# JuliaParallel/DistributedArrays.jl

Hardware: NVIDIA H100
Metric: GB/s for map! and sum on Float32 DArray (higher is better)
Workload: dtype f32

## Files before the change

### distributedarrays.jl_b200/_broadcast.py

```python
from __future__ import annotations

import ctypes as C
import struct
from typing import Callable, List, Optional, Sequence, Tuple

import numpy as np

from builtins import any as builtins_any

from . import _lib
from ._darray import B200Array, DArray, dab_dtype, darray, makelocal
from .layout import shape_of
from .runtime import close_remote_reads, open_remote_reads, runtime

_RANK = {"bool": 0, "i32": 1, "i64": 2, "i128": 3, "f32": 4, "f64": 5}


class _TagTypes(dict):

    def __missing__(self, tag):
        raise _lib.UnsupportedError(_lib.ERR_UNSUPPORTED, f"values of type {tag} have no array element type on the GPU backend "
                                    "(Int128 is served as the value type of mapreduce(f, op, d) only)")


_NPT = _TagTypes({"bool": np.dtype(np.bool_), "i32": np.dtype(np.int32), "i64": np.dtype(np.int64), "f32": np.dtype(np.float32),
                  "f64": np.dtype(np.float64), "c64": np.dtype(np.complex64), "c128": np.dtype(np.complex128)})
_TAG = {v: k for k, v in _NPT.items()}
SLICE_TRACING = [0]
_CT = {"bool": "bool", "i32": "int", "i64": "long long", "i128": "i128", "f32": "float", "f64": "double", "c64": "jl_c64", "c128": "jl_c128"}
_COMP = {"c64": "f32", "c128": "f64"}
_CPLX_OF = {"f32": "c64", "f64": "c128"}


def is_ctag(t: str) -> bool:
    return t in _COMP


def tag_of(dtype) -> str:
    dt = np.dtype(dtype)
    if dt not in _TAG:
        raise _lib.UnsupportedError(_lib.ERR_UNSUPPORTED, f"element type {dt} not served by the GPU backend")
    return _TAG[dt]


def promote(a: str, b: str) -> str:
    if a == b:
        return a
    if is_ctag(a) or is_ctag(b):
        if "i128" in (a, b):
            raise _lib.UnsupportedError(_lib.ERR_UNSUPPORTED, "Int128 values mixed with complex values are not served")
        return _CPLX_OF[promote(_COMP.get(a, a), _COMP.get(b, b))]
    if "f" in a[0] + b[0]:
        fl = [t for t in (a, b) if t[0] == "f"]
        return "f64" if "f64" in fl else "f32"
    return a if _RANK[a] >= _RANK[b] else b


class Expr:

    __slots__ = ("op", "args", "jt", "val", "weak")
    __array_ufunc__ = None

    def __init__(self, op, args=(), jt="f64", val=None, weak=False):
        self.op, self.args, self.jt, self.val, self.weak = op, tuple(args), jt, val, weak
# ... 354 lines not shown
        return unop("inv", inner(x))
    f.__name__ = name
    return f


def _mk_of_inv(name, outer):
    def f(x):
        if not isinstance(x, Expr):
            raise TypeError(f"dab.{name} is for use inside broadcast/map kernels")
        return outer(unop("inv", x))
    f.__name__ = name
    return f


sec, csc, cot = _mk_inv_of("sec", cos), _mk_inv_of("csc", sin), _mk_inv_of("cot", tan)
sech, csch, coth = _mk_inv_of("sech", cosh), _mk_inv_of("csch", sinh), _mk_inv_of("coth", tanh)
asec, acsc, acot = _mk_of_inv("asec", acos), _mk_of_inv("acsc", asin), _mk_of_inv("acot", atan)
asech, acsch, acoth = _mk_of_inv("asech", acosh), _mk_of_inv("acsch", asinh), _mk_of_inv("acoth", atanh)


def _float_of(x: Expr) -> Expr:
    return x if x.jt[0] == "f" else convert(x, "f64")


def deg2rad(x):
    x = _float_of(Expr.wrap(x))
    t = _NPT[x.jt].type
    return binop("mul", x, Expr("const", (), x.jt, float(t(np.pi) / t(180))))


def rad2deg(x):
    x = _float_of(Expr.wrap(x))
    t = _NPT[x.jt].type
    return binop("mul", x, Expr("const", (), x.jt, float(t(180) / t(np.pi))))


def jl_max(a, b):
    return binop("max", Expr.wrap(a), Expr.wrap(b))


def jl_min(a, b):
    return binop("min", Expr.wrap(a), Expr.wrap(b))


def mod(a, b):
    return binop("mod", Expr.wrap(a), Expr.wrap(b))


def rem(a, b):
    return binop("rem", Expr.wrap(a), Expr.wrap(b))


def trace(f: Callable, arg_tags: Sequence[str]) -> Expr:
    syms = [Expr("arg", (), t, k) for k, t in enumerate(arg_tags)]
    return Expr.wrap(f(*syms))


_FN2 = {"add": "jl_add", "sub": "jl_sub", "mul": "jl_mul", "div": "jl_div", "rem": "jl_rem", "mod": "jl_mod", "idiv": "jl_idiv",
        "max": "jl_max", "min": "jl_min", "pow": "jl_pow", "and": "jl_and", "or": "jl_or", "xor": "jl_xor", "lt": "jl_lt", "le": "jl_le",
        "gt": "jl_gt", "ge": "jl_ge", "eq": "jl_eq", "ne": "jl_ne", "x_shl": "jl_x_shl", "x_shr": "jl_x_shr"}
_FN2.update({"m_copysign": "jl_m_copysign", "m_powi": "jl_m_powi"})
_FN2.update({"m_" + c: "jl_m_" + c for c in ("lt", "le", "gt", "ge", "eq", "ne")})


def _lit(jt: str, v) -> str:
    if jt == "f32":
        return "__int_as_float((int)0x%08x)" % struct.unpack("<I", struct.pack("<f", float(v)))[0]
    if jt == "f64":
        return "__longlong_as_double((long long)0x%016xULL)" % struct.unpack("<Q", struct.pack("<d", float(v)))[0]
    if is_ctag(jt):
        z = complex(v)
        return "%s(%s, %s)" % (_CT[jt], _lit(_COMP[jt], z.real), _lit(_COMP[jt], z.imag))
    if jt == "i32":
        return "((int)%d)" % int(v)
    if jt == "i64":
        return "((long long)%dLL)" % int(v)
    if jt == "i128":
        v = int(v) % (1 << 128)
        return "((i128)(((u128)0x%016xULL << 64) | (u128)0x%016xULL))" % (v >> 64, v & ((1 << 64) - 1))
    return "true" if v else "false"


def codegen(e: Expr) -> str:
    if e.op == "arg":
        return f"a{e.val}"
    if e.op == "const":
        return _lit(e.jt, e.val)
    if e.op == "convert":
        if is_ctag(e.jt):
            return f"{_CT[e.jt]}({codegen(e.args[0])})"
        return f"(({_CT[e.jt]})({codegen(e.args[0])}))"
    if e.op == "complex":
        return f"{_CT[e.jt]}({codegen(e.args[0])}, {codegen(e.args[1])})"
    if e.op == "ifelse":
        return f"(({codegen(e.args[0])}) ? ({codegen(e.args[1])}) : ({codegen(e.args[2])}))"
    if e.op in _FN2:
        return f"{_FN2[e.op]}({codegen(e.args[0])}, {codegen(e.args[1])})"
    return f"jl_{e.op}({codegen(e.args[0])})"


_UN = {"abs": _lib.MAP_ABS, "abs2": _lib.MAP_ABS2, "neg": _lib.MAP_NEG, "sqrt": _lib.MAP_SQRT, "inv": _lib.MAP_INV,
       "floor": _lib.MAP_FLOOR, "ceil": _lib.MAP_CEIL, "sign": _lib.MAP_SIGN}
_BIN = {"add": _lib.ADD, "sub": _lib.SUB, "mul": _lib.MUL, "div": _lib.DIV, "rem": _lib.REM, "max": _lib.BMAX, "min": _lib.BMIN,
        "mod": _lib.MOD, "idiv": _lib.IDIV, "and": _lib.AND, "or": _lib.OR, "xor": _lib.XOR}


def _is_arg(e: Expr, k=None):
    return e.op == "arg" and (k is None or e.val == k)


def match_affine(e: Expr):
    def lin(t):
        if _is_arg(t, 0):
            return 1
        if t.op == "mul":
            l, r = t.args
            if l.op == "const" and _is_arg(r, 0):
                return l.val
            if r.op == "const" and _is_arg(l, 0):
                return r.val
        return None

    if e.op == "add":
        l, r = e.args
        if r.op == "const" and lin(l) is not None:
            return lin(l), r.val
        if l.op == "const" and lin(r) is not None:
            return lin(r), l.val
    return None


def _pad4(v, fill=1):
    v = list(v)
    if len(v) > 4:
        raise _lib.UnsupportedError(_lib.ERR_UNSUPPORTED, "broadcast whose dimensions do not collapse to 4 groups (see collapse_dims) is not served")
    return v + [fill] * (4 - len(v))


def collapse_dims(out_shape, arg_shapes):
    nd = len(out_shape)
    shapes = [tuple(int(v) for v in sh) + (1,) * (nd - len(sh)) for sh in arg_shapes]
    groups: List[Tuple[int, List[int]]] = []
    for d in range(nd):
        o = int(out_shape[d])
        ext = [sh[d] for sh in shapes]
        for e, sh in zip(ext, arg_shapes):
            if e != o and e != 1:
                raise _lib.DimensionMismatch(_lib.ERR_DIM_MISMATCH, f"arrays could not be broadcast: {tuple(sh)} vs {tuple(out_shape)}")
        if o == 1:
            continue
        if groups:
            po, pext = groups[-1]
            if all((pe == po and e == o) or (pe == 1 and e == 1) for pe, e in zip(pext, ext)):
                groups[-1] = (po * o, [pe * e for pe, e in zip(pext, ext)])
                continue
        groups.append((o, ext))
    if not groups:
        groups = [(1, [1] * len(shapes))]
    return tuple(g[0] for g in groups), [tuple(g[1][k] for g in groups) for k in range(len(shapes))]


def _dense_strides(shape):
    s, out = 1, []
    for d in shape:
        out.append(s)
        s *= int(d)
    return out


class LocalArg:

    def __init__(self, arr: Optional[B200Array] = None, scalar=None, tag: str = "f64", temp: bool = False):
        self.arr, self.scalar, self.tag, self.temp = arr, scalar, tag, temp


def run_local(rt, expr: Expr, out: B200Array, largs: List[LocalArg]):
    n = out.size
    if n == 0:
        return
    out_tag = tag_of(out.dtype)
    full = [a for a in largs if a.arr is not None]
    same = all(a.arr.shape == out.shape or a.arr.size == n and _squeeze(a.arr.shape) == _squeeze(out.shape) for a in full)
    ctx = rt.ctx
    code = dab_dtype(out.dtype)
    rt.last_kernel = "fixed"
    cplx = uses_complex(expr) or builtins_any(is_ctag(a.tag) for a in largs)
    if same and not cplx and expr.jt == out_tag and out_tag != "bool":
        x0 = largs[0] if largs and largs[0].arr is not None and largs[0].tag == out_tag else None
        if x0 is not None and all(_only_arg0(expr)):
            ab = match_affine(expr)
            if ab is not None:
                a = np.asarray(ab[0], dtype=out.dtype)
                b = np.asarray(ab[1], dtype=out.dtype)
                _lib.call("dab_affine", ctx, code, C.c_void_p(out.ptr), C.c_void_p(x0.arr.ptr), C.c_void_p(a.ctypes.data),
                          C.c_void_p(b.ctypes.data), n)
                rt.last_kernel = "dab_affine"
                return
            if expr.op in _UN and _is_arg(expr.args[0], 0):
                _lib.call("dab_unary", ctx, code, _UN[expr.op], C.c_void_p(out.ptr), C.c_void_p(x0.arr.ptr), n)
                return
            if _is_arg(expr, 0):
                _lib.call("dab_unary", ctx, code, _lib.MAP_ID, C.c_void_p(out.ptr), C.c_void_p(x0.arr.ptr), n)
                return
        if expr.op in _BIN and len(expr.args) == 2 and not (expr.op == "div" and out_tag[0] != "f"):
            l, r = expr.args
            la = largs[l.val] if l.op == "arg" else None
            ra = largs[r.val] if r.op == "arg" else None

            def arr_ok(e, a):
                return e.op == "arg" and a is not None and a.arr is not None and a.tag == out_tag

            def sc_val(e, a):
                if e.op == "const" and e.jt == out_tag:
                    return e.val
                if e.op == "arg" and a is not None and a.arr is None and a.tag == out_tag:
                    return a.scalar
                return None

            if arr_ok(l, la) and arr_ok(r, ra):
                _lib.call("dab_binary", ctx, code, _BIN[expr.op], C.c_void_p(out.ptr), C.c_void_p(la.arr.ptr), C.c_void_p(ra.arr.ptr), n)
                return
            if arr_ok(l, la) and sc_val(r, ra) is not None:
                s = np.asarray(sc_val(r, ra), dtype=out.dtype)
                _lib.call("dab_binary_scalar", ctx, code, _BIN[expr.op], C.c_void_p(out.ptr), C.c_void_p(la.arr.ptr), C.c_void_p(s.ctypes.data), 0, n)
                return
            if arr_ok(r, ra) and sc_val(l, la) is not None:
                s = np.asarray(sc_val(l, la), dtype=out.dtype)
                _lib.call("dab_binary_scalar", ctx, code, _BIN[expr.op], C.c_void_p(out.ptr), C.c_void_p(ra.arr.ptr), C.c_void_p(s.ctypes.data), 1, n)
                return
    if expr.op == "const" and expr.jt == out_tag:
        v = np.asarray(expr.val, dtype=out.dtype)
        _lib.call("dab_fill", ctx, code, C.c_void_p(out.ptr), n, C.c_void_p(v.ctypes.data))
        return
    rt.last_kernel = "dab_broadcast_expr"
    if uses_tag(expr, "i128"):
        raise _lib.UnsupportedError(_lib.ERR_UNSUPPORTED, "Int128 values are served inside mapreduce(f, op, d) only, not in a broadcast")
    if expr.jt[0] == "f" and out_tag[0] not in "fc":
        raise _lib.UnsupportedError(_lib.ERR_UNSUPPORTED, f"broadcast of {expr.jt} values into a {out_tag} destination (InexactError semantics) is not served")
    if is_ctag(expr.jt) and not is_ctag(out_tag):
        raise _lib.UnsupportedError(_lib.ERR_UNSUPPORTED, f"broadcast of {expr.jt} values into a {out_tag} destination (InexactError semantics) is not served")
    expr, largs = split_c128_scalars(expr, largs)
    src = codegen(convert(expr, out_tag)).encode()
    oshape_nd, ashapes = tuple(out.shape), {k: tuple(a.arr.shape) for k, a in enumerate(largs) if a.arr is not None}
    if len(oshape_nd) > 4 or any(len(sh) > 4 for sh in ashapes.values()):
        keys = sorted(ashapes)
        oshape_nd, coll = collapse_dims(oshape_nd, [ashapes[k] for k in keys])
        ashapes = dict(zip(keys, coll))
    oshape = _pad4(oshape_nd)
    nargs = len(largs)
    if nargs > 8:
# ... 62 lines not shown
        ext = 1
        for s in shapes:
            v = s[k] if k < len(s) else 1
            if v != 1:
                if ext != 1 and ext != v:
                    raise _lib.DimensionMismatch(_lib.ERR_DIM_MISMATCH, f"arrays could not be broadcast to a common size: {shapes}")
                ext = v
        out.append(ext)
    return tuple(out)


def _arg_tag(a) -> str:
    if isinstance(a, (DArray,)):
        return tag_of(a.dtype)
    if isinstance(a, np.ndarray) and a.ndim > 0:
        return tag_of(a.dtype)
    return Expr.wrap(a.item() if isinstance(a, np.ndarray) else a).jt


def _bcview(arg_dims: Sequence[int], I) -> Tuple:
    out = []
    for k, s in enumerate(arg_dims):
        if s == 1:
            out.append((1, 1))
        elif k < len(I):
            lo, hi = I[k]
            if not (1 <= lo and hi <= s):
                raise _lib.DimensionMismatch(_lib.ERR_DIM_MISMATCH, "broadcast view could not be constructed")
            out.append((lo, hi))
        else:
            out.append((1, s))
    return tuple(out)


def _localise(rt, a, I, pid) -> LocalArg:
    if isinstance(a, DArray):
        view = _bcview(a.dims, I)
        arr = makelocal(a, view, pid)
        return LocalArg(arr, None, tag_of(a.dtype), temp=arr is not a.chunks.get(pid))
    if isinstance(a, np.ndarray) and a.ndim > 0:
        view = _bcview(a.shape, I)
        sl = a[tuple(slice(lo - 1, hi) for lo, hi in view)]
        return LocalArg(B200Array.from_numpy(rt, sl), None, tag_of(a.dtype), temp=True)
    e = Expr.wrap(a.item() if isinstance(a, np.ndarray) else a)
    return LocalArg(None, e.val, e.jt)


def _remote_args(dest_layout, args) -> List[DArray]:
    return [a for a in args if isinstance(a, DArray) and not (a.layout.pids == dest_layout.pids and a.layout.indices == dest_layout.indices)]


def _broadcast_chunks(dest: DArray, expr: Expr, args) -> DArray:
    rt = dest.rt
    fenced = open_remote_reads(rt, _remote_args(dest.layout, args), "host")
    for pid, out in dest.chunks.items():
        I = dest.layout.localindices(pid)
        largs = [_localise(rt, a, I, pid) for a in args]
        run_local(rt, expr, out, largs)
        for la in largs:
            if la.temp and la.arr is not None:
                la.arr.free()
    close_remote_reads(rt, fenced, "host")
    return dest


def _materialise_views(args):
    from ._darray import SubDArray
    out, temps = [], []
    for a in args:
        if isinstance(a, SubDArray):
            a = a.to_darray()
            temps.append(a)
        out.append(a)
    return out, temps


def broadcast_into(dest: DArray, f: Callable, *args) -> DArray:
    args, _views = _materialise_views(args)
    try:
        return _broadcast_into(dest, f, *args)
    finally:
        for v in _views:
            v.close()


def _broadcast_into(dest: DArray, f: Callable, *args) -> DArray:
    shapes = [a.dims if isinstance(a, DArray) else (a.shape if isinstance(a, np.ndarray) else ()) for a in args]
    for shp in shapes:
        for k, s in enumerate(shp):
            want = dest.dims[k] if k < len(dest.dims) else 1
            if s != 1 and s != want:
                raise _lib.DimensionMismatch(_lib.ERR_DIM_MISMATCH, f"destination axes {dest.dims} are not compatible with source axes {tuple(shp)}")
    expr = trace(f, [_arg_tag(a) for a in args])
    return _broadcast_chunks(dest, expr, args)


def broadcast(f: Callable, *args, rt=None) -> DArray:
    args, _views = _materialise_views(args)
    try:
        return _broadcast(f, *args, rt=rt)
    finally:
        for v in _views:
            v.close()


def _broadcast(f: Callable, *args, rt=None) -> DArray:
    rt = rt or next((a.rt for a in args if isinstance(a, DArray)), None) or runtime()
    shapes = [a.dims if isinstance(a, DArray) else (a.shape if isinstance(a, np.ndarray) else ()) for a in args]
    dims = _bc_shape(shapes)
    expr = trace(f, [_arg_tag(a) for a in args])
    out_dt = _NPT[expr.jt]
    dest = darray(lambda I: B200Array.empty(rt, shape_of(I), out_dt), dims, dtype=out_dt, rt=rt)
    return _broadcast_chunks(dest, expr, args)


def copy(d: DArray) -> DArray:
    from ._darray import similar
    return _broadcast_into(similar(d), lambda x: x, d)


# ... 68 lines not shown
```

### distributedarrays.jl_b200/_darray.py

```python
from __future__ import annotations

import ctypes as C
import itertools
import weakref
from typing import Callable, Dict, List, Optional, Sequence, Tuple

import numpy as np

from . import _lib
from .layout import Layout, Range, default_procs, layout_from_chunk_shapes, make_layout, rlen, shape_of, slab_plan
from .runtime import Runtime, close_remote_reads, open_remote_reads, runtime

_DT = {np.dtype(np.float32): _lib.F32, np.dtype(np.float64): _lib.F64, np.dtype(np.int32): _lib.I32,
       np.dtype(np.int64): _lib.I64, np.dtype(np.bool_): _lib.U8,
       np.dtype(np.complex64): _lib.C64, np.dtype(np.complex128): _lib.C128}
_NP = {_lib.F32: np.dtype(np.float32), _lib.F64: np.dtype(np.float64), _lib.I32: np.dtype(np.int32),
       _lib.I64: np.dtype(np.int64), _lib.U8: np.dtype(np.bool_), _lib.C64: np.dtype(np.complex64), _lib.C128: np.dtype(np.complex128)}


def dab_dtype(dt) -> int:
    dt = np.dtype(dt)
    if dt not in _DT:
        raise _lib.UnsupportedError(_lib.ERR_UNSUPPORTED, f"element type {dt} is not served by the GPU backend (no host fallback)")
    return _DT[dt]


def np_dtype(code: int) -> np.dtype:
    return _NP[code]


def is_complex(dt) -> bool:
    return np.dtype(dt).kind == "c"


def component_dtype(dt) -> np.dtype:
    dt = np.dtype(dt)
    return {np.dtype(np.complex64): np.dtype(np.float32), np.dtype(np.complex128): np.dtype(np.float64)}.get(dt, dt)


_allowscalar = [True]


def allowscalar(flag: bool = True):
    _allowscalar[0] = bool(flag)


class B200Array:

    __slots__ = ("rt", "ptr", "shape", "dtype", "_own", "_keep", "_temp")

    def __init__(self, rt: Runtime, ptr: int, shape: Sequence[int], dtype, own: bool = True, keep=None, temp: bool = False):
        self.rt, self.ptr, self.shape, self.dtype = rt, int(ptr), tuple(int(s) for s in shape), np.dtype(dtype)
        self._own, self._keep, self._temp = own, keep, temp

    @classmethod
    def empty(cls, rt: Runtime, shape: Sequence[int], dtype, temp: bool = False) -> "B200Array":
        dtype = np.dtype(dtype)
        n = int(np.prod(shape)) if len(shape) else 1
        ptr = rt.alloc_temp(n * dtype.itemsize) if temp else rt.alloc(n * dtype.itemsize)
        return cls(rt, ptr, shape, dtype, temp=temp)

    @classmethod
    def from_numpy(cls, rt: Runtime, a: np.ndarray) -> "B200Array":
        a = np.asarray(a)
        dab_dtype(a.dtype)
        out = cls.empty(rt, a.shape, a.dtype)
        out.copy_from_host(a)
        return out

    @property
    def size(self) -> int:
        return int(np.prod(self.shape)) if len(self.shape) else 1

    @property
    def nbytes(self) -> int:
        return self.size * self.dtype.itemsize

    @property
    def ndim(self) -> int:
        return len(self.shape)

    def copy_from_host(self, a: np.ndarray, sync: bool = True):
        a = np.asarray(a, dtype=self.dtype)
        if tuple(a.shape) != self.shape:
            raise _lib.DimensionMismatch(_lib.ERR_DIM_MISMATCH, f"host array {a.shape} vs chunk {self.shape}")
        if self.size == 0:
            return
        if not a.flags.f_contiguous:
            if a.ndim == 2 and a.strides[0] == a.itemsize and a.strides[1] > 0:
                _lib.call("dab_h2d_2d", self.rt.ctx, C.c_void_p(self.ptr), a.shape[0] * a.itemsize, C.c_void_p(a.ctypes.data),
                          a.strides[1], a.shape[0] * a.itemsize, a.shape[1])
                if sync:
                    self.rt.sync()
                return
            a = np.asfortranarray(a)
        _lib.call("dab_h2d", self.rt.ctx, C.c_void_p(self.ptr), C.c_void_p(a.ctypes.data), self.nbytes)
        if sync:
            self.rt.sync()

    def to_numpy(self) -> np.ndarray:
        out = np.empty(self.shape, dtype=self.dtype, order="F")
        if self.size:
            _lib.call("dab_d2h", self.rt.ctx, C.c_void_p(out.ctypes.data), C.c_void_p(self.ptr), self.nbytes)
            self.rt.sync()
        return out

    def free(self):
        if self._own and self.ptr:
            if self._temp:
                self.rt.free_temp(self.ptr)
            else:
                self.rt.free(self.ptr)
        self.ptr = 0

    def __repr__(self):
        return f"B200Array({self.dtype}, {self.shape}, ptr=0x{self.ptr:x}, dev={self.rt.device})"


def pinned_empty(rt: Runtime, shape, dtype) -> np.ndarray:
    dtype = np.dtype(dtype)
    n = int(np.prod(shape)) if len(shape) else 1
    p = C.c_void_p()
    _lib.call("dab_host_alloc", rt.ctx, max(1, n * dtype.itemsize), C.byref(p))
    buf = (C.c_char * max(1, n * dtype.itemsize)).from_address(p.value)
    arr = np.frombuffer(buf, dtype=dtype, count=n).reshape(shape, order="F")
# ... 627 lines not shown
```

### distributedarrays.jl_b200/_mapreduce.py

```python
from __future__ import annotations

import builtins
import ctypes as C
import operator
from itertools import accumulate
from typing import Callable, Dict, Optional, Sequence, Tuple

import numpy as np

from . import _lib
from ._broadcast import Expr, broadcast, is_ctag, tag_of, trace, _NPT
from ._darray import B200Array, DArray, component_dtype, dab_dtype, is_complex, np_dtype
from .layout import Layout, ravel, reduction_passes, shape_of, unravel
from .runtime import close_remote_reads, deliver, exchange_stacks, open_remote_reads

_OPS = {"+": _lib.SUM, "add": _lib.SUM, "sum": _lib.SUM, "*": _lib.PROD, "mul": _lib.PROD, "prod": _lib.PROD, "max": _lib.MAX,
        "min": _lib.MIN}
_OPF = {operator.add: _lib.SUM, operator.mul: _lib.PROD, builtins.max: _lib.MAX, builtins.min: _lib.MIN, np.add: _lib.SUM,
        np.multiply: _lib.PROD, np.maximum: _lib.MAX, np.minimum: _lib.MIN}


def _op_code(op) -> int:
    if isinstance(op, str) and op in _OPS:
        return _OPS[op]
    if op in _OPF:
        return _OPF[op]
    raise _lib.UnsupportedError(_lib.ERR_UNSUPPORTED, f"reduction operator {op!r} is not served by a kernel (no host fallback)")


_CMPMAP = {"eq": _lib.MAP_EQ, "ne": _lib.MAP_NE, "lt": _lib.MAP_LT, "le": _lib.MAP_LE, "gt": _lib.MAP_GT, "ge": _lib.MAP_GE}
_FLIP = {"lt": "gt", "le": "ge", "gt": "lt", "ge": "le", "eq": "eq", "ne": "ne"}


def classify_map(f: Optional[Callable], dtype) -> Tuple[Optional[int], Optional[np.ndarray], Optional[Expr]]:
    if f is None:
        return _lib.MAP_ID, None, None
    tag = tag_of(dtype)
    e = trace(f, [tag])
    if e.op == "arg":
        return _lib.MAP_ID, None, e
    if is_ctag(tag):
        if len(e.args) == 1 and e.args[0].op == "arg":
            code = {"abs": _lib.MAP_ABS, "abs2": _lib.MAP_ABS2, "neg": _lib.MAP_NEG, "isnan": _lib.MAP_ISNAN}.get(e.op)
            if code is not None:
                return code, None, e
        return None, None, e
    if e.jt == tag and len(e.args) == 1 and e.args[0].op == "arg":
        code = {"abs": _lib.MAP_ABS, "abs2": _lib.MAP_ABS2, "neg": _lib.MAP_NEG}.get(e.op)
        if code is not None:
            return code, None, e
    if e.op == "mul" and e.jt == tag and builtins.all(a.op == "arg" for a in e.args):
        return _lib.MAP_ABS2, None, e
    if e.op in _CMPMAP:
        l, r = e.args

        def unpromote(side, const):
            if side.op == "convert" and side.args[0].op == "arg" and side.args[0].jt == tag and const.op == "const":
                c = const.val
                if tag == "f32" and const.jt == "f64" and float(np.float32(c)) == c:
                    return side.args[0], Expr("const", (), tag, c)
                if tag in ("i32", "i64") and const.jt in ("i64",) and side.jt == "i64":
                    return side.args[0], Expr("const", (), tag, c) if -2**31 <= c < 2**31 or tag == "i64" else (side, const)
            return side, const

        l, r = unpromote(l, r)
        r, l = unpromote(r, l)
        if l.op == "arg" and r.op == "const" and l.jt == tag:
            return _CMPMAP[e.op], np.asarray(r.val, dtype=np.dtype(dtype)), e
        if r.op == "arg" and l.op == "const" and r.jt == tag:
            return _CMPMAP[_FLIP[e.op]], np.asarray(l.val, dtype=np.dtype(dtype)), e
    if e.op == "isnan" and e.args[0].op == "arg":
        return _lib.MAP_ISNAN, None, e
    return None, None, e


def _result_dtype(dtype, op: int, mapc: int) -> np.dtype:
    out = C.c_int32()
    _lib.check(_lib.lib().dab_reduce_result_dtype(dab_dtype(dtype), op, mapc, C.byref(out)))
    return np.dtype(np.int64) if out.value == _lib.I64 else np_dtype(out.value)




def _gather_slots(d: DArray, launch: Callable[[int, B200Array, int], None]) -> np.ndarray:
    rt = d.rt
    wpr = rt.workers_per_rank
    slots = B200Array.empty(rt, (16 * wpr,), np.uint8, temp=True)
    try:
        for pid, ch in d.chunks.items():
            launch(pid, ch, slots.ptr + 16 * ((pid - 1) % wpr))
        if rt.world > 1:
            allslots = B200Array.empty(rt, (16 * wpr * rt.world,), np.uint8, temp=True)
            _lib.call("dab_allgather", rt.ctx, C.c_void_p(slots.ptr), C.c_void_p(allslots.ptr), 16 * wpr)
            host = allslots.to_numpy()
            allslots.free()
        else:
            host = slots.to_numpy()
    finally:
        rt.sync()
        slots.free()
    return host.view(np.uint8)


def _fold(host: np.ndarray, pids: Sequence[int], rdt: np.dtype, op: int):
    vals = np.empty(len(pids), dtype=rdt)
    for i, pid in enumerate(pids):
        vals[i] = host[16 * (pid - 1):16 * (pid - 1) + rdt.itemsize].view(rdt)[0]
    out = np.zeros(1, dtype=rdt)
    rcode = _lib.I64 if rdt == np.dtype(np.int64) else dab_dtype(rdt)
    _lib.check(_lib.lib().dab_combine_ordered(rcode, op, C.c_void_p(vals.ctypes.data), len(pids), C.c_void_p(out.ctypes.data)))
    return out[0], vals


def _int128(b: bytes) -> int:
    return int.from_bytes(b, "little", signed=True)


def wrap128(v: int) -> int:
    v &= (1 << 128) - 1
    return v - (1 << 128) if v >> 127 else v


def fold128(vals: Sequence[int], op: int) -> int:
    acc = vals[0]
    for v in vals[1:]:
        acc = wrap128(acc + v) if op == _lib.SUM else wrap128(acc * v) if op == _lib.PROD else (max(acc, v) if op == _lib.MAX else min(acc, v))
    return acc


# ... 520 lines not shown
```

### distributedarrays.jl_b200/csrc/dab_comm.cu

```cuda
#include <dlfcn.h>
#include <nccl.h>

#include "dab_common.cuh"
#include "dab_scalar_ops.cuh"

namespace {

struct NcclApi {
    void* handle = nullptr;
    ncclResult_t (*GetUniqueId)(ncclUniqueId*) = nullptr;
    ncclResult_t (*CommInitRank)(ncclComm_t*, int, ncclUniqueId, int) = nullptr;
    ncclResult_t (*CommDestroy)(ncclComm_t) = nullptr;
    ncclResult_t (*AllGather)(const void*, void*, size_t, ncclDataType_t, ncclComm_t, cudaStream_t) = nullptr;
    ncclResult_t (*AllReduce)(const void*, void*, size_t, ncclDataType_t, ncclRedOp_t, ncclComm_t, cudaStream_t) = nullptr;
    ncclResult_t (*Send)(const void*, size_t, ncclDataType_t, int, ncclComm_t, cudaStream_t) = nullptr;
    ncclResult_t (*Recv)(void*, size_t, ncclDataType_t, int, ncclComm_t, cudaStream_t) = nullptr;
    ncclResult_t (*GroupStart)() = nullptr;
    ncclResult_t (*GroupEnd)() = nullptr;
    const char* (*GetErrorString)(ncclResult_t) = nullptr;
    const char* (*GetLastError)(ncclComm_t) = nullptr;
    bool ok = false;
    char why[256] = "";
};

// ... 152 lines not shown
    }
    ncclRedOp_t ro;
    switch (op) {
        case DAB_SUM: ro = ncclSum; break;
        case DAB_PROD: ro = ncclProd; break;
        case DAB_MAX: ro = ncclMax; break;
        case DAB_MIN: ro = ncclMin; break;
        default: return dab_fail(ctx, DAB_ERR_ARG, "dab_allreduce: bad op %d", op);
    }
    DAB_NCCL(ctx, api.AllReduce(send_dev, recv_dev, count, dt, ro, (ncclComm_t)ctx->comm, ctx->stream));
    ctx->launches++;
    return DAB_OK;
}

int32_t dab_group_start(dab_ctx* ctx) {
    DAB_ENTER(ctx);
    NEED_COMM(ctx);
    DAB_NCCL(ctx, api.GroupStart());
    return DAB_OK;
}
int32_t dab_group_end(dab_ctx* ctx) {
    DAB_ENTER(ctx);
    NEED_COMM(ctx);
    DAB_NCCL(ctx, api.GroupEnd());
    ctx->launches++;
    return DAB_OK;
}
int32_t dab_send(dab_ctx* ctx, const void* send_dev, size_t nbytes, int32_t peer) {
    DAB_ENTER(ctx);
    NEED_COMM(ctx);
    DAB_NCCL(ctx, api.Send(send_dev, nbytes, ncclInt8, peer, (ncclComm_t)ctx->comm, ctx->stream));
    return DAB_OK;
}
int32_t dab_recv(dab_ctx* ctx, void* recv_dev, size_t nbytes, int32_t peer) {
    DAB_ENTER(ctx);
    NEED_COMM(ctx);
    DAB_NCCL(ctx, api.Recv(recv_dev, nbytes, ncclInt8, peer, (ncclComm_t)ctx->comm, ctx->stream));
    return DAB_OK;
}

int32_t dab_mapreduce_all(dab_ctx* ctx, int32_t dtype, int32_t op, int32_t map, const void* map_param, const void* x, size_t n,
                          void* out_host) {
    DAB_ENTER_NOFLUSH(ctx);
    int32_t rdt;
    if (!out_host || op == DAB_EXTREMA || dab_reduce_result_dtype(dtype, op, map, &rdt) != DAB_OK) {
        DAB_FLUSH(ctx);
        DAB_REQUIRE(ctx, out_host, DAB_ERR_ARG, "dab_mapreduce_all: null out");
        if (op == DAB_EXTREMA) return dab_fail(ctx, DAB_ERR_UNSUPPORTED, "dab_mapreduce_all: extrema combines through dab_reduce + dab_allgather");
        return dab_fail(ctx, DAB_ERR_ARG, "bad dtype/op");
    }
    const bool cplx = rdt == DAB_C64 || rdt == DAB_C128;
    if ((ctx->mbox_ranks > 1 || !ctx->comm || ctx->nranks == 1) && n > 0 && !cplx) {
        ctx->fuse_op = op;
        int32_t st = dab_reduce(ctx, dtype, op, map, map_param, x, n, ctx->result_slot);
        ctx->fuse_op = -1;
        if (st != DAB_OK) return st;
        DAB_CUDA(ctx, cudaStreamSynchronize(ctx->stream));
        const volatile unsigned long long* h = (const volatile unsigned long long*)ctx->host_slot;
        if (h[1] != 0) return dab_fail(ctx, DAB_ERR_NCCL, "fused combine timed out waiting for a peer's chunk result (did every rank call?)");
        unsigned long long bits = h[0];
        memset(out_host, 0, 8);
        memcpy(out_host, &bits, dab_dtype_size(rdt));
        return DAB_OK;
    }
    if (cplx && ctx->mbox_ranks > 1 && !ctx->comm) {
        DAB_FLUSH(ctx);
        return dab_fail(ctx, DAB_ERR_UNSUPPORTED, "dab_mapreduce_all: a complex result across %d ranks needs the NCCL communicator "
                        "(the mailbox combine carries 8-byte results)", ctx->mbox_ranks);
    }
    int32_t st = dab_reduce(ctx, dtype, op, map, map_param, x, n, ctx->result_slot);
    if (st != DAB_OK) return st;
    const int P = ctx->comm ? ctx->nranks : 1;
    const void* src = ctx->result_slot;
    if (P > 1) {
        NEED_COMM(ctx);
        DAB_NCCL(ctx, api.AllGather(ctx->result_slot, ctx->gather_slots, 16, ncclInt8, (ncclComm_t)ctx->comm, ctx->stream));
        ctx->launches++;
        src = ctx->gather_slots;
    }
    DAB_CUDA(ctx, cudaMemcpyAsync(ctx->host_slot, src, (size_t)P * 16, cudaMemcpyDeviceToHost, ctx->stream));
    DAB_CUDA(ctx, cudaStreamSynchronize(ctx->stream));
    unsigned char tmp[DAB_MAX_RANKS * 16];
    size_t es = dab_dtype_size(rdt);
    for (int i = 0; i < P; ++i) memcpy(tmp + (size_t)i * es, (const char*)ctx->host_slot + (size_t)i * 16, es);
    unsigned char res[16] = {0};
    st = dab_combine_ordered(rdt, op, tmp, (size_t)P, res);
    if (st != DAB_OK) return dab_fail(ctx, st, "%s", dab_last_error(nullptr));
    memset(out_host, 0, es > 8 ? es : 8);
    memcpy(out_host, res, es);
    return DAB_OK;
}

int32_t dab_mailbox_create(dab_ctx* ctx, void* handle64) {
    DAB_ENTER(ctx);
    DAB_REQUIRE(ctx, handle64, DAB_ERR_ARG, "dab_mailbox_create: null handle");
    if (!ctx->mailbox) {
        DAB_CUDA(ctx, cudaMalloc(&ctx->mailbox, DAB_MBOX_BYTES));
        DAB_CUDA(ctx, cudaMemset(ctx->mailbox, 0, DAB_MBOX_BYTES));
    }
    cudaIpcMemHandle_t h;
    DAB_CUDA(ctx, cudaIpcGetMemHandle(&h, ctx->mailbox));
    memcpy(handle64, &h, 64);
    return DAB_OK;
}

int32_t dab_mailbox_attach(dab_ctx* ctx, const void* handles, int32_t rank, int32_t nranks) {
    DAB_ENTER(ctx);
    DAB_REQUIRE(ctx, handles && nranks >= 1 && nranks <= DAB_MAX_RANKS && rank >= 0 && rank < nranks, DAB_ERR_ARG, "dab_mailbox_attach: bad arguments");
    DAB_REQUIRE(ctx, ctx->mailbox, DAB_ERR_ARG, "dab_mailbox_attach: call dab_mailbox_create first");
    DAB_REQUIRE(ctx, ctx->mbox_ranks == 0, DAB_ERR_ARG, "mailboxes already attached");
    for (int j = 0; j < nranks; ++j) {
        if (j == rank) {
            ctx->peer_mbox_host[j] = ctx->mailbox;
            continue;
        }
        cudaIpcMemHandle_t h;
        memcpy(&h, (const char*)handles + (size_t)j * 64, 64);
        DAB_CUDA(ctx, cudaIpcOpenMemHandle(&ctx->peer_mbox_host[j], h, cudaIpcMemLazyEnablePeerAccess));
    }
    DAB_CUDA(ctx, cudaMalloc((void**)&ctx->peer_mbox_dev, sizeof(void*) * DAB_MAX_RANKS));
    DAB_CUDA(ctx, cudaMemcpy(ctx->peer_mbox_dev, ctx->peer_mbox_host, sizeof(void*) * nranks, cudaMemcpyHostToDevice));
    ctx->rank = rank;
    ctx->mbox_ranks = nranks;
// ... 94 lines not shown
```

### distributedarrays.jl_b200/csrc/dab_common.cuh

```cuda
#pragma once
#include <cuda_runtime.h>

#include <cstdint>
#include <cstdio>
#include <cstring>

#include "../../include/dab200.h"

#define DAB_MAX_REDUCE_BLOCKS 262144
#define DAB_SLOT_BYTES 64
#define DAB_MAX_RANKS 64

struct dab_pending_affine {
    int active;
    int32_t dtype;
    void* y;
    const void* x;
    size_t n;
    unsigned char a[8], b[8];
};

struct dab_ctx {
    int device;
    int sm_count;
// ... 31 lines not shown
    long long opt_combine_timeout_ms;
    long long opt_gemm_kc;
    int opt_gemm_rawhi;
    int opt_gemm_simt;
    int opt_gemv_phase;
    int opt_gemv_t_cols;
    int opt_gemv_t_waves;
    int opt_spmv_group;
    int opt_ew_tma;
    dab_pending_affine pending;
    int defer_off;
    char err[512];
};

extern thread_local char dab_tls_err[512];

int32_t dab_fail(dab_ctx* ctx, int32_t status, const char* fmt, ...);
int32_t dab_fail_cuda(dab_ctx* ctx, cudaError_t e, const char* what, const char* file, int line);

#define DAB_CUDA(ctx, call)                                                             \
    do {                                                                                \
        cudaError_t e__ = (call);                                                       \
        if (e__ != cudaSuccess) return dab_fail_cuda((ctx), e__, #call, __FILE__, __LINE__); \
    } while (0)

#define DAB_REQUIRE(ctx, cond, status, ...)                          \
    do {                                                             \
        if (!(cond)) return dab_fail((ctx), (status), __VA_ARGS__);  \
    } while (0)

int32_t dab_flush_pending(dab_ctx* ctx);

#define DAB_FLUSH(ctx)                                    \
    do {                                                  \
        if ((ctx)->pending.active) {                      \
            int32_t st__ = dab_flush_pending(ctx);        \
            if (st__ != DAB_OK) return st__;              \
        }                                                 \
    } while (0)

#define DAB_ENTER(ctx)                                                      \
    do {                                                                    \
        if ((ctx) == nullptr) return dab_fail(nullptr, DAB_ERR_ARG, "null ctx"); \
        DAB_CUDA((ctx), cudaSetDevice((ctx)->device));                      \
        DAB_FLUSH(ctx);                                                     \
    } while (0)

#define DAB_ENTER_NOFLUSH(ctx)                                              \
    do {                                                                    \
        if ((ctx) == nullptr) return dab_fail(nullptr, DAB_ERR_ARG, "null ctx"); \
        DAB_CUDA((ctx), cudaSetDevice((ctx)->device));                      \
    } while (0)

#define DAB_LAUNCHED(ctx)                          \
    do {                                           \
        (ctx)->launches++;                         \
        DAB_CUDA((ctx), cudaGetLastError());       \
    } while (0)

int32_t dab_scratch_grow(dab_ctx* ctx, void** buf, size_t* have, size_t bytes, bool zero);

static inline size_t dab_dtype_size(int32_t dt) {
    switch (dt) {
        case DAB_F32: return 4;
        case DAB_F64: return 8;
        case DAB_I32: return 4;
        case DAB_I64: return 8;
        case DAB_U8: return 1;
        case DAB_C64: return 8;
        case DAB_C128: return 16;
        default: return 0;
    }
}

#define DAB_MBOX_SLOT 32
#define DAB_MBOX_BARRIER_OFFSET (2 * DAB_MAX_RANKS * DAB_MBOX_SLOT)
#define DAB_MBOX_BYTES (DAB_MBOX_BARRIER_OFFSET + DAB_MAX_RANKS * 8)
struct FusedComm {
    void* const* peers;
    void* host_out;
    unsigned long long seq;
    unsigned long long timeout_ns;
    int rank, nranks, op;
};

__device__ __forceinline__ unsigned long long dab_globaltimer_ns() {
    unsigned long long t;
    asm volatile("mov.u64 %0, %globaltimer;" : "=l"(t));
    return t;
}
__device__ __forceinline__ int4 ld_stream(const int4* p) { return __ldcs(p); }
__device__ __forceinline__ void st_stream(int4* p, int4 v) { __stcs(p, v); }

template <typename T>
struct alignas(16) Pack {
    static constexpr int N = 16 / sizeof(T);
    T v[N];
};

template <typename T>
struct alignas(2 * sizeof(T)) Cplx {
    T re, im;
};

template <typename T>
__device__ __forceinline__ Pack<T> as_pack(int4 r) {
// ... 32 lines not shown
```

### distributedarrays.jl_b200/csrc/dab_reduce.cu

```cuda
#include <type_traits>

#include <cmath>

#include "dab_reduce_traits.cuh"

namespace {

struct NoStore {
    template <typename T>
    __device__ __forceinline__ void vec(Pack<T>&, size_t) const {}
    template <typename T>
    __device__ __forceinline__ T scalar(T v, size_t) const { return v; }
};
template <typename T>
struct AffineStore {
    AffineF<T> f;
    T* y;
    int4* yv;
    __device__ __forceinline__ void vec(Pack<T>& p, size_t i) const {
#pragma unroll
        for (int k = 0; k < Pack<T>::N; ++k) p.v[k] = f(p.v[k]);
        st_stream(yv + i, as_int4(p));
    }
    __device__ __forceinline__ T scalar(T v, size_t i) const {
// ... 342 lines not shown
                memcpy(buf, one, 16);
            } else {
                long long one = 1;
                memcpy(buf, &one, 8);
            }
            if (flt) {
                double one = 1.0;
                memcpy(buf + 8, &one, 8);
            }
            break;
        default: return dab_fail(ctx, DAB_ERR_EMPTY, "reducing over an empty collection is not allowed");
    }
    memcpy((char*)ctx->host_slot + DAB_MAX_RANKS * 16, buf, 16);
    DAB_CUDA(ctx, cudaMemcpyAsync(out_dev, (char*)ctx->host_slot + DAB_MAX_RANKS * 16, 16, cudaMemcpyHostToDevice, ctx->stream));
    DAB_CUDA(ctx, cudaStreamSynchronize(ctx->stream));
    return DAB_OK;
}

}

extern "C" {

int32_t dab_reduce_result_dtype(int32_t dtype, int32_t op, int32_t map, int32_t* out_dtype) {
    if (!out_dtype) return DAB_ERR_ARG;
    if (dtype == DAB_C64 || dtype == DAB_C128) {
        const int32_t comp = dtype == DAB_C64 ? DAB_F32 : DAB_F64;
        const bool id = map == DAB_MAP_ID || map == DAB_MAP_NEG, mag = map == DAB_MAP_ABS || map == DAB_MAP_ABS2;
        const bool pred = map == DAB_MAP_NONZERO || map == DAB_MAP_ISNAN;
        if (id && (op == DAB_SUM || op == DAB_PROD)) *out_dtype = dtype;
        else if (mag && (op == DAB_SUM || op == DAB_MAX || op == DAB_MIN)) *out_dtype = comp;
        else if (pred && (op == DAB_SUM || op == DAB_COUNT || op == DAB_ALL || op == DAB_ANY)) *out_dtype = DAB_I64;
        else return dab_fail(nullptr, DAB_ERR_UNSUPPORTED, "op %d with map %d is not served for complex dtype %d", op, map, dtype);
        return DAB_OK;
    }
    const bool pred = map >= DAB_MAP_EQ;
    switch (op) {
        case DAB_SUM:
        case DAB_PROD:
            *out_dtype = (!pred && (dtype == DAB_F32 || dtype == DAB_F64)) ? dtype : DAB_I64;
            return DAB_OK;
        case DAB_MAX:
        case DAB_MIN:
        case DAB_EXTREMA: *out_dtype = dtype; return DAB_OK;
        case DAB_ALL:
        case DAB_ANY:
        case DAB_COUNT: *out_dtype = DAB_I64; return DAB_OK;
        default: return DAB_ERR_ARG;
    }
}

int32_t dab_reduce(dab_ctx* ctx, int32_t dtype, int32_t op, int32_t map, const void* map_param, const void* x, size_t n,
                   void* out_dev) {
    DAB_ENTER_NOFLUSH(ctx);
    if (out_dev && consumes_pending(ctx, dtype, op, map, x, n)) {
        const dab_pending_affine p = ctx->pending;
        ctx->pending.active = 0;
        switch (dtype) {
            case DAB_F32: return reduce_pending_affine<float>(ctx, op, p, out_dev);
            case DAB_F64: return reduce_pending_affine<double>(ctx, op, p, out_dev);
            case DAB_I32: return reduce_pending_affine<int32_t>(ctx, op, p, out_dev);
            default: return reduce_pending_affine<long long>(ctx, op, p, out_dev);
        }
    }
    DAB_FLUSH(ctx);
    DAB_REQUIRE(ctx, out_dev && (x || n == 0), DAB_ERR_ARG, "dab_reduce: null pointer");
    DAB_REQUIRE(ctx, op >= DAB_SUM && op <= DAB_EXTREMA, DAB_ERR_ARG, "dab_reduce: bad op %d", op);
    if (dtype == DAB_C64 || dtype == DAB_C128) {
        int32_t rdt;
        if (dab_reduce_result_dtype(dtype, op, map, &rdt) != DAB_OK)
            return dab_fail(ctx, DAB_ERR_UNSUPPORTED, "dab_reduce: op %d with map %d is not served for complex dtype %d (no host fallback)", op,
                            map, dtype);
        if (n == 0) return empty_result(ctx, map == DAB_MAP_ABS || map == DAB_MAP_ABS2 ? rdt : dtype, op, out_dev);
        if (dtype == DAB_C64) return reduce_c<float>(ctx, dtype, op, map, (const Cplx<float>*)x, n, out_dev);
        return reduce_c<double>(ctx, dtype, op, map, (const Cplx<double>*)x, n, out_dev);
    }
    if (n == 0) return empty_result(ctx, dtype, op, out_dev);
    switch (dtype) {
        case DAB_F32: return reduce_t<float>(ctx, op, map, map_param, (const float*)x, n, out_dev);
        case DAB_F64: return reduce_t<double>(ctx, op, map, map_param, (const double*)x, n, out_dev);
        case DAB_I32: return reduce_t<int32_t>(ctx, op, map, map_param, (const int32_t*)x, n, out_dev);
        case DAB_I64: return reduce_t<long long>(ctx, op, map, map_param, (const long long*)x, n, out_dev);
        case DAB_U8: return reduce_u8(ctx, op, map, (const uint8_t*)x, n, out_dev);
        default: return dab_fail(ctx, DAB_ERR_ARG, "dab_reduce: bad dtype %d", dtype);
    }
}

int32_t dab_reduce_host(dab_ctx* ctx, int32_t dtype, int32_t op, int32_t map, const void* map_param, const void* x, size_t n,
                        void* out_host) {
    DAB_ENTER_NOFLUSH(ctx);
    if (!out_host) {
        DAB_FLUSH(ctx);
        return dab_fail(ctx, DAB_ERR_ARG, "dab_reduce_host: null out");
    }
    int32_t st = dab_reduce(ctx, dtype, op, map, map_param, x, n, ctx->result_slot);
    if (st != DAB_OK) return st;
    DAB_CUDA(ctx, cudaMemcpyAsync(ctx->host_slot, ctx->result_slot, 16, cudaMemcpyDeviceToHost, ctx->stream));
    DAB_CUDA(ctx, cudaStreamSynchronize(ctx->stream));
    memcpy(out_host, ctx->host_slot, 16);
    return DAB_OK;
}

int32_t dab_combine_ordered(int32_t rdt, int32_t op, const void* partials, size_t p, void* out) {
    if (!partials || !out) return dab_fail(nullptr, DAB_ERR_ARG, "dab_combine_ordered: null pointer");
    if (p == 0) return dab_fail(nullptr, DAB_ERR_EMPTY, "reducing over an empty collection is not allowed");
#define FOLD(T, EXPR)                          \
    {                                          \
        const T* v = (const T*)partials;       \
        T a = v[0];                            \
        for (size_t i = 1; i < p; ++i) {       \
            T b = v[i];                        \
            a = (EXPR);                        \
        }                                      \
        *(T*)out = a;                          \
        return DAB_OK;                         \
    }
    auto fmax_jl = [](auto a, auto b) {
        using T = decltype(a);
        if (a != a || b != b) return (T)NAN;
        if (a == b) return std::signbit(a) ? b : a;
        return a > b ? a : b;
    };
    auto fmin_jl = [](auto a, auto b) {
        using T = decltype(a);
        if (a != a || b != b) return (T)NAN;
        if (a == b) return std::signbit(a) ? a : b;
        return a < b ? a : b;
    };
    switch (rdt) {
        case DAB_F32:
            switch (op) {
                case DAB_SUM: {
                    const float* v = (const float*)partials;
                    volatile float a = v[0];
                    for (size_t i = 1; i < p; ++i) a = a + v[i];
                    *(float*)out = a;
                    return DAB_OK;
                }
                case DAB_PROD: {
                    const float* v = (const float*)partials;
                    volatile float a = v[0];
                    for (size_t i = 1; i < p; ++i) a = a * v[i];
                    *(float*)out = a;
                    return DAB_OK;
                }
                case DAB_MAX: FOLD(float, fmax_jl(a, b))
                case DAB_MIN: FOLD(float, fmin_jl(a, b))
                default: break;
// ... 85 lines not shown
```

Baseline: 4008.

## Trim host-side overhead in broadcast and reduce dispatch paths

Caches traced expressions for closures whose captured values are plain numbers, and tries the affine kernel before the costlier complex-usage scan. It also skips the remote-read fence on a single rank, short-circuits view materialisation, memoises result dtype lookups and uses math.prod for size. A dab_reduce_entered entry avoids re-entering the context guard on nested calls. The aim is to cut Python and C entry overhead per map!/sum call, at the cost of added cache-key logic that could mis-key closures.

Measured after the change: 4122 (median of 6 runs). 2.8% higher.

```diff
diff --git a/distributedarrays.jl_b200/_broadcast.py b/distributedarrays.jl_b200/_broadcast.py
--- a/distributedarrays.jl_b200/_broadcast.py
+++ b/distributedarrays.jl_b200/_broadcast.py
@@ -2,6 +2,8 @@
 
 import ctypes as C
 import struct
+from collections import OrderedDict
+from types import CodeType, FunctionType
 from typing import Callable, List, Optional, Sequence, Tuple
 
 import numpy as np
@@ -9,7 +11,7 @@
 from builtins import any as builtins_any
 
 from . import _lib
-from ._darray import B200Array, DArray, dab_dtype, darray, makelocal
+from ._darray import B200Array, DArray, SubDArray, dab_dtype, darray, makelocal
 from .layout import shape_of
 from .runtime import close_remote_reads, open_remote_reads, runtime
 
@@ -470,8 +472,49 @@
 
 
 def trace(f: Callable, arg_tags: Sequence[str]) -> Expr:
+    key = _closed_key(f, arg_tags)
+    if key is not None:
+        e = _TRACES.get(key)
+        if e is not None:
+            _TRACES.move_to_end(key)
+            return e
     syms = [Expr("arg", (), t, k) for k, t in enumerate(arg_tags)]
-    return Expr.wrap(f(*syms))
+    e = Expr.wrap(f(*syms))
+    if key is not None:
+        _TRACES[key] = e
+        if len(_TRACES) > _TRACES_MAX:
+            _TRACES.popitem(last=False)
+    return e
+
+
+_TRACES: "OrderedDict[tuple, Expr]" = OrderedDict()
+_TRACES_MAX = 64
+_CELL_TYPES = frozenset({bool, int, float, complex} | {t for t in np.sctypeDict.values() if issubclass(t, (np.number, np.bool_))})
+
+
+def _closed_key(f, arg_tags) -> Optional[tuple]:
+    if type(f) is not FunctionType or f.__defaults__ or f.__kwdefaults__ or SLICE_TRACING[0]:
+        return None
+    code = f.__code__
+    if code.co_names or builtins_any(isinstance(c, CodeType) for c in code.co_consts):
+        return None
+    cells = []
+    for cell in f.__closure__ or ():
+        try:
+            v = cell.cell_contents
+        except ValueError:
+            return None
+        t = type(v)
+        if t not in _CELL_TYPES:
+            return None
+        if t is float:
+            v = struct.pack("<d", v)
+        elif t is complex:
+            v = struct.pack("<dd", v.real, v.imag)
+        elif t is not int and t is not bool:
+            v = v.tobytes()
+        cells.append((t, v))
+    return (code, tuple(arg_tags), tuple(cells))
 
 
 _FN2 = {"add": "jl_add", "sub": "jl_sub", "mul": "jl_mul", "div": "jl_div", "rem": "jl_rem", "mod": "jl_mod", "idiv": "jl_idiv",
@@ -530,17 +573,21 @@
 def match_affine(e: Expr):
     def lin(t):
         if _is_arg(t, 0):
-            return 1
-        if t.op == "mul":
+            return None if is_ctag(t.jt) else 1
+        if t.op == "mul" and not is_ctag(t.jt):
             l, r = t.args
+            if is_ctag(l.jt) or is_ctag(r.jt):
+                return None
             if l.op == "const" and _is_arg(r, 0):
                 return l.val
             if r.op == "const" and _is_arg(l, 0):
                 return r.val
         return None
 
-    if e.op == "add":
+    if e.op == "add" and not is_ctag(e.jt):
         l, r = e.args
+        if is_ctag(l.jt) or is_ctag(r.jt):
+            return None
         if r.op == "const" and lin(l) is not None:
             return lin(l), r.val
         if l.op == "const" and lin(r) is not None:
@@ -602,18 +649,21 @@
     ctx = rt.ctx
     code = dab_dtype(out.dtype)
     rt.last_kernel = "fixed"
-    cplx = uses_complex(expr) or builtins_any(is_ctag(a.tag) for a in largs)
-    if same and not cplx and expr.jt == out_tag and out_tag != "bool":
-        x0 = largs[0] if largs and largs[0].arr is not None and largs[0].tag == out_tag else None
+    cplx_args = builtins_any(is_ctag(a.tag) for a in largs)
+    fixed = same and expr.jt == out_tag and out_tag != "bool"
+    x0 = largs[0] if largs and largs[0].arr is not None and largs[0].tag == out_tag else None
+    if fixed and x0 is not None and not cplx_args:
+        ab = match_affine(expr)
+        if ab is not None:
+            a = np.asarray(ab[0], dtype=out.dtype)
+            b = np.asarray(ab[1], dtype=out.dtype)
+            _lib.call("dab_affine", ctx, code, C.c_void_p(out.ptr), C.c_void_p(x0.arr.ptr), C.c_void_p(a.ctypes.data),
+                      C.c_void_p(b.ctypes.data), n)
+            rt.last_kernel = "dab_affine"
+            return
+    cplx = cplx_args or uses_complex(expr)
+    if fixed and not cplx:
         if x0 is not None and all(_only_arg0(expr)):
-            ab = match_affine(expr)
-            if ab is not None:
-                a = np.asarray(ab[0], dtype=out.dtype)
-                b = np.asarray(ab[1], dtype=out.dtype)
-                _lib.call("dab_affine", ctx, code, C.c_void_p(out.ptr), C.c_void_p(x0.arr.ptr), C.c_void_p(a.ctypes.data),
-                          C.c_void_p(b.ctypes.data), n)
-                rt.last_kernel = "dab_affine"
-                return
             if expr.op in _UN and _is_arg(expr.args[0], 0):
                 _lib.call("dab_unary", ctx, code, _UN[expr.op], C.c_void_p(out.ptr), C.c_void_p(x0.arr.ptr), n)
                 return
@@ -782,7 +832,7 @@
 
 def _broadcast_chunks(dest: DArray, expr: Expr, args) -> DArray:
     rt = dest.rt
-    fenced = open_remote_reads(rt, _remote_args(dest.layout, args), "host")
+    fenced = rt.world > 1 and open_remote_reads(rt, _remote_args(dest.layout, args), "host")
     for pid, out in dest.chunks.items():
         I = dest.layout.localindices(pid)
         largs = [_localise(rt, a, I, pid) for a in args]
@@ -795,7 +845,8 @@
 
 
 def _materialise_views(args):
-    from ._darray import SubDArray
+    if not builtins_any(isinstance(a, SubDArray) for a in args):
+        return args, ()
     out, temps = [], []
     for a in args:
         if isinstance(a, SubDArray):
diff --git a/distributedarrays.jl_b200/_darray.py b/distributedarrays.jl_b200/_darray.py
--- a/distributedarrays.jl_b200/_darray.py
+++ b/distributedarrays.jl_b200/_darray.py
@@ -2,6 +2,7 @@
 
 import ctypes as C
 import itertools
+import math
 import weakref
 from typing import Callable, Dict, List, Optional, Sequence, Tuple
 
@@ -70,7 +71,7 @@
 
     @property
     def size(self) -> int:
-        return int(np.prod(self.shape)) if len(self.shape) else 1
+        return math.prod(self.shape)
 
     @property
     def nbytes(self) -> int:
diff --git a/distributedarrays.jl_b200/_mapreduce.py b/distributedarrays.jl_b200/_mapreduce.py
--- a/distributedarrays.jl_b200/_mapreduce.py
+++ b/distributedarrays.jl_b200/_mapreduce.py
@@ -2,6 +2,7 @@
 
 import builtins
 import ctypes as C
+import functools
 import operator
 from itertools import accumulate
 from typing import Callable, Dict, Optional, Sequence, Tuple
@@ -74,7 +75,8 @@
     return None, None, e
 
 
-def _result_dtype(dtype, op: int, mapc: int) -> np.dtype:
+@functools.lru_cache(maxsize=None)
+def _result_dtype(dtype: np.dtype, op: int, mapc: int) -> np.dtype:
     out = C.c_int32()
     _lib.check(_lib.lib().dab_reduce_result_dtype(dab_dtype(dtype), op, mapc, C.byref(out)))
     return np.dtype(np.int64) if out.value == _lib.I64 else np_dtype(out.value)
diff --git a/distributedarrays.jl_b200/csrc/dab_comm.cu b/distributedarrays.jl_b200/csrc/dab_comm.cu
--- a/distributedarrays.jl_b200/csrc/dab_comm.cu
+++ b/distributedarrays.jl_b200/csrc/dab_comm.cu
@@ -228,7 +228,7 @@
     const bool cplx = rdt == DAB_C64 || rdt == DAB_C128;
     if ((ctx->mbox_ranks > 1 || !ctx->comm || ctx->nranks == 1) && n > 0 && !cplx) {
         ctx->fuse_op = op;
-        int32_t st = dab_reduce(ctx, dtype, op, map, map_param, x, n, ctx->result_slot);
+        int32_t st = dab_reduce_entered(ctx, dtype, op, map, map_param, x, n, ctx->result_slot);
         ctx->fuse_op = -1;
         if (st != DAB_OK) return st;
         DAB_CUDA(ctx, cudaStreamSynchronize(ctx->stream));
@@ -244,7 +244,7 @@
         return dab_fail(ctx, DAB_ERR_UNSUPPORTED, "dab_mapreduce_all: a complex result across %d ranks needs the NCCL communicator "
                         "(the mailbox combine carries 8-byte results)", ctx->mbox_ranks);
     }
-    int32_t st = dab_reduce(ctx, dtype, op, map, map_param, x, n, ctx->result_slot);
+    int32_t st = dab_reduce_entered(ctx, dtype, op, map, map_param, x, n, ctx->result_slot);
     if (st != DAB_OK) return st;
     const int P = ctx->comm ? ctx->nranks : 1;
     const void* src = ctx->result_slot;
diff --git a/distributedarrays.jl_b200/csrc/dab_common.cuh b/distributedarrays.jl_b200/csrc/dab_common.cuh
--- a/distributedarrays.jl_b200/csrc/dab_common.cuh
+++ b/distributedarrays.jl_b200/csrc/dab_common.cuh
@@ -107,6 +107,9 @@
         DAB_CUDA((ctx), cudaSetDevice((ctx)->device));                      \
     } while (0)
 
+int32_t dab_reduce_entered(dab_ctx* ctx, int32_t dtype, int32_t op, int32_t map, const void* map_param, const void* x, size_t n,
+                           void* out_dev);
+
 #define DAB_LAUNCHED(ctx)                          \
     do {                                           \
         (ctx)->launches++;                         \
diff --git a/distributedarrays.jl_b200/csrc/dab_reduce.cu b/distributedarrays.jl_b200/csrc/dab_reduce.cu
--- a/distributedarrays.jl_b200/csrc/dab_reduce.cu
+++ b/distributedarrays.jl_b200/csrc/dab_reduce.cu
@@ -418,6 +418,13 @@
 int32_t dab_reduce(dab_ctx* ctx, int32_t dtype, int32_t op, int32_t map, const void* map_param, const void* x, size_t n,
                    void* out_dev) {
     DAB_ENTER_NOFLUSH(ctx);
+    return dab_reduce_entered(ctx, dtype, op, map, map_param, x, n, out_dev);
+}
+
+}
+
+int32_t dab_reduce_entered(dab_ctx* ctx, int32_t dtype, int32_t op, int32_t map, const void* map_param, const void* x, size_t n,
+                           void* out_dev) {
     if (out_dev && consumes_pending(ctx, dtype, op, map, x, n)) {
         const dab_pending_affine p = ctx->pending;
         ctx->pending.active = 0;
@@ -451,6 +458,8 @@
     }
 }
 
+extern "C" {
+
 int32_t dab_reduce_host(dab_ctx* ctx, int32_t dtype, int32_t op, int32_t map, const void* map_param, const void* x, size_t n,
                         void* out_host) {
     DAB_ENTER_NOFLUSH(ctx);
@@ -458,7 +467,7 @@
         DAB_FLUSH(ctx);
         return dab_fail(ctx, DAB_ERR_ARG, "dab_reduce_host: null out");
     }
-    int32_t st = dab_reduce(ctx, dtype, op, map, map_param, x, n, ctx->result_slot);
+    int32_t st = dab_reduce_entered(ctx, dtype, op, map, map_param, x, n, ctx->result_slot);
     if (st != DAB_OK) return st;
     DAB_CUDA(ctx, cudaMemcpyAsync(ctx->host_slot, ctx->result_slot, 16, cudaMemcpyDeviceToHost, ctx->stream));
     DAB_CUDA(ctx, cudaStreamSynchronize(ctx->stream));
```
